# MAGPIE-ICL/synthPy

Hardware: AMD Instinct MI355X
Metric: ray-steps/sec (+ rays/sec to detector), 1e7 rays x 512^3 volume (higher is better)
Workload: dtype f64

## Files before the change

### include/synthray.h

```cpp
#ifndef SYNTHRAY_H
#define SYNTHRAY_H

#include <stddef.h>
#include <stdint.h>

#ifdef __cplusplus
extern "C" {
#endif

#define SR_OK 0
#define SR_ERR_INVALID (-1)
#define SR_ERR_HIP (-2)
#define SR_ERR_RCCL (-3)
#define SR_ERR_STATE (-4)

typedef struct sr_volume sr_volume;
typedef struct sr_rays sr_rays;
typedef struct sr_image sr_image;
typedef struct sr_comm sr_comm;

int sr_init(int device);
int sr_device_count(void);
int sr_synchronize(void);
int sr_device_memory(int64_t *free_bytes, int64_t *total_bytes);
// ... 176 lines not shown

int sr_ray_to_jones(const double *sf, int64_t n_rays, double extent, int probing_axis, int row_order,
                    double *rf, double *Jf);

int sr_rays_create(sr_rays **out, int64_t n_rays);
int sr_rays_upload(sr_rays *r, const double *s0);
int sr_rays_upload_part(sr_rays *r, const double *s0, int64_t n, int64_t first, int last);
int sr_rays_generate(sr_rays *r, int beam_type, double size_a, double size_b, double divergence, double ne_extent,
                     int probing_axis, uint64_t seed, uint64_t first_ray);
int sr_rays_trace(sr_rays *r, const sr_volume *v, const sr_trace_params *p, sr_trace_stats *stats);
int sr_rays_trace_stats(sr_rays *r, sr_trace_stats *stats);

int sr_rays_tile_segments(const sr_rays *r);
int sr_rays_tile_records(const sr_rays *r);
int sr_rays_launch_order(const sr_rays *r, uint32_t *order);
int sr_rays_set_count(sr_rays *r, int64_t n);
double sr_tile_min_density(void);
int sr_rays_download(const sr_rays *r, double *sf, double *rf, double *Jf);
int sr_rays_download_s0(const sr_rays *r, double *s0);
int sr_rays_error_bound(const sr_rays *r, float *bound);
int64_t sr_rays_count(const sr_rays *r);
int sr_rays_handoff_download(const sr_rays *r, double *rec);
int sr_rays_set_bbox(sr_rays *r, const double *bbox);
int sr_rays_get_bbox(const sr_rays *r, double *bbox, int *known);
int sr_rays_handoff_upload(sr_rays *r, const double *rec);
int sr_rays_handoff_send(sr_rays *r, sr_comm *comm, int peer);
int sr_rays_handoff_recv(sr_rays *r, sr_comm *comm, int peer);
void sr_rays_destroy(sr_rays *r);

enum {
// ... 86 lines not shown
```

### synthpy_amd/_ffi.py

```python
from __future__ import annotations

import ctypes as C
import os

import numpy as np

_HERE = os.path.dirname(os.path.abspath(__file__))
LIB_PATH = os.environ.get("SYNTHRAY_LIB") or os.path.join(_HERE, "libsynthray.so")


class SynthrayError(RuntimeError):
    """A libsynthray call returned a negative status."""


class Optic(C.Structure):
    _fields_ = [("op", C.c_int32), ("iarg", C.c_int32), ("a", C.c_double), ("b", C.c_double)]


class TraceParams(C.Structure):
    _fields_ = [("t_end", C.c_double), ("extent", C.c_double), ("dt", C.c_double), ("probing_axis", C.c_int32),
                ("row_order", C.c_int32), ("substeps", C.c_int32), ("sort_rays", C.c_int32), ("precision", C.c_int32),
                ("handoff", C.c_int32)]


# ... 127 lines not shown
    "sr_trace": (_i, [_vp, _vp, _i64, C.POINTER(TraceParams), _vp, _vp, _vp, C.POINTER(TraceStats)]),
    "sr_ray_to_jones": (_i, [_vp, _i64, _d, _i, _i, _vp, _vp]),
    "sr_rays_create": (_i, [_pp, _i64]),
    "sr_rays_download_s0": (_i, [_vp, _vp]),
    "sr_rays_error_bound": (_i, [_vp, _vp]),
    "sr_rays_generate": (_i, [_vp, _i, _d, _d, _d, _d, _i, C.c_uint64, C.c_uint64]),
    "sr_rays_upload": (_i, [_vp, _vp]),
    "sr_rays_upload_part": (_i, [_vp, _vp, _i64, _i64, _i]),
    "sr_rays_trace": (_i, [_vp, _vp, C.POINTER(TraceParams), C.POINTER(TraceStats)]),
    "sr_release_caches": (_i, []),
    "sr_rays_trace_stats": (_i, [_vp, C.POINTER(TraceStats)]),
    "sr_rays_tile_segments": (_i, [_vp]),
    "sr_tile_min_density": (_d, []),
    "sr_rays_tile_records": (_i, [_vp]),
    "sr_rays_launch_order": (_i, [_vp, _vp]),
    "sr_rays_set_count": (_i, [_vp, _i64]),
    "sr_rays_set_bbox": (_i, [_vp, _vp]),
    "sr_rays_get_bbox": (_i, [_vp, _vp, C.POINTER(C.c_int)]),
    "sr_rays_download": (_i, [_vp, _vp, _vp, _vp]),
    "sr_rays_count": (_i64, [_vp]),
    "sr_rays_destroy": (None, [_vp]),
    "sr_optics": (_i, [C.POINTER(Optic), _i, _d, _i64, _vp, _vp, _vp, _vp]),
    "sr_hist2d": (_i, [_vp, _vp, _i64, _i, _i, _d, _d, _d, _d, _vp]),
    "sr_interferogram": (_i, [_vp, _vp, _vp, _i64, _i, _i, _d, _d, _d, _d, _vp, _vp]),
    "sr_interfere_ref_beam": (_i, [_vp, _vp, _i64, _d, _d, _vp]),
    "sr_image_create": (_i, [_pp, _i, _i, _i, _d, _d, _d, _d]),
    "sr_image_zero": (_i, [_vp]),
    "sr_image_download": (_i, [_vp, _vp]),
    "sr_image_amplitude": (_i, [_vp, _vp]),
    "sr_image_counts_f64": (_i, [_vp, _vp]),
# ... 58 lines not shown
```

### synthpy_amd/csrc/common.hpp

```cpp
#pragma once
#include <hip/hip_runtime.h>

#include <algorithm>
#include <cmath>
#include <cstdarg>
#include <cstdint>
#include <cstdio>
#include <initializer_list>
#include <map>
#include <string>
#include <type_traits>
#include <vector>

#include "synthray.h"

namespace sr {

constexpr double kC = 299792458.0;

void set_error(const char *fmt, ...);
int fail(int code, const char *fmt, ...);

#define SR_HIP(call)                                                                         \
  do {                                                                                       \
// ... 178 lines not shown
  bool bbox_given = false;
  double *s0 = nullptr;
  double *sf = nullptr;
  double *rf = nullptr;
  double *Jf = nullptr;
  uint32_t *perm = nullptr;
  uint32_t *keys = nullptr;
  uint32_t *bins = nullptr;
  uint32_t *sort_tmp = nullptr;
  int64_t bins_cap = 0;
  uint32_t *fb_list = nullptr;
  unsigned long long *counters = nullptr;
  double *rec = nullptr;
  double *rec2 = nullptr;
  uint32_t *order2 = nullptr;
  double *strag_rec = nullptr;
  unsigned long long *strag_snap = nullptr;
  int strag_snap_cap = 0;
  bool have_s0 = false, traced = false, sorted = false, have_rec = false;
  bool have_order = false;
  bool counters_carry = false;
  int tile_segs = 0;
  int tile_segs_run = 0;
  bool tile_rec = false;
  float *guard = nullptr;
  const sr_volume *last_vol = nullptr;
  sr_trace_params last_p{};
  void *guard_set = nullptr;
  std::vector<char> guard_set_host;
  bool guard_live = false;
// ... 68 lines not shown
```

### synthpy_amd/csrc/trace.hip

```cpp
#include <algorithm>
#include <cmath>
#include <cstdlib>
#include <cstring>

#include "common.hpp"

namespace {

struct VolDev {
  const float4 *P;
  const float *L;
  const double *g[3];
  const double *rg[3];
  int na, nb, nc;
  double omega;
  const double *K;
  const double *Q;
  double verdet;
  int64_t OS;
  const double *R;
};

constexpr int64_t kSC = 8;
__device__ __forceinline__ int64_t col8(const VolDev &V, int ib, int ic) { return ((int64_t)ib * V.nc + ic) * 8; }
__device__ __forceinline__ int64_t koff(const VolDev &V, int k) { return (int64_t)(k >> 3) * V.OS + (k & 7); }

__device__ __forceinline__ void lds_dma16(const char *src, unsigned lane_off, unsigned dst) {
#ifdef SR_TILE_EXP_DMA_SADDR
  unsigned keep;
  asm volatile("s_mov_b32 %0, m0\n\ts_mov_b32 m0, %3\n\ts_nop 0\n\tglobal_load_lds_dwordx4 %1, %2\n\ts_mov_b32 m0, %0"
               : "=&s"(keep)
               : "v"(lane_off), "s"(src), "s"(dst)
               : "memory");
#else
  __builtin_amdgcn_global_load_lds((const __attribute__((address_space(1))) void *)(src + lane_off),
// ... 620 lines not shown
  V.P = v->P;
  V.L = v->L;
  for (int k = 0; k < 3; ++k) {
    V.g[k] = v->g[k];
    V.rg[k] = v->rg[k];
  }
  V.na = v->na;
  V.nb = v->nb;
  V.nc = v->nc;
  V.omega = v->omega;
  V.K = v->K;
  V.Q = v->Q;
  V.verdet = v->verdet;
  V.OS = (int64_t)v->nb * v->nc * 8;
  V.R = v->R;
  return V;
}

int bin_rays(sr_rays *r, int64_t N, int lo_bits, int n_coarse, uint32_t *out, hipStream_t st) {
  SR_CHECK(lo_bits <= 11 && n_coarse <= kBinMaxDigits + 1, "lateral grid too large for the LDS counters of the ray binning");
  const unsigned n_wg = (unsigned)((N + kBinTile - 1) / kBinTile);
  const int64_t ncount = (int64_t)n_coarse * n_wg;
  const int64_t nsb = (ncount + kScanPerBlock - 1) / kScanPerBlock;
  if (r->bins_cap < ncount + nsb) {
    sr::dev_free(r->bins);
    r->bins = nullptr;
    r->bins_cap = 0;
    int rc = sr::dev_alloc(&r->bins, (size_t)(ncount + nsb));
    if (rc) return rc;
    r->bins_cap = ncount + nsb;
// ... 4 lines not shown
  }
  uint32_t *sums = r->bins + ncount, *tkeys = r->sort_tmp, *trays = r->sort_tmp + N;
  hipLaunchKernelGGL(k_bin_count, dim3(n_wg), dim3(256), 0, st, (const uint32_t *)r->keys, N, lo_bits, n_coarse, r->bins, n_wg);
  hipLaunchKernelGGL(k_scan_blocks, dim3((unsigned)nsb), dim3(256), 0, st, r->bins, ncount, sums);
  hipLaunchKernelGGL(k_scan, dim3(1), dim3(1024), 0, st, sums, nsb);
  hipLaunchKernelGGL(k_scan_add, dim3(sr::grid_for(ncount, 256)), dim3(256), 0, st, r->bins, ncount, (const uint32_t *)sums);
  hipLaunchKernelGGL(k_bin_coarse, dim3(n_wg), dim3(256), 0, st, (const uint32_t *)r->keys, N, lo_bits, n_coarse,
                     (const uint32_t *)r->bins, n_wg, tkeys, trays);
  hipLaunchKernelGGL(k_bin_fine, dim3((unsigned)n_coarse), dim3(1024), 0, st, (const uint32_t *)tkeys, (const uint32_t *)trays, N,
                     lo_bits, n_coarse, (const uint32_t *)r->bins, n_wg, out);
  return SR_OK;
}

int bin_by_band(sr_rays *r, const sr_volume *v, const TileGeom &g, const double *rec, uint32_t *out, hipStream_t st) {
  const int64_t N = r->n;
  const int64_t n_bands = (v->nb - 1 + g.band - 1) / g.band;
  const int64_t n_keys = n_bands * (int64_t)(v->nc - 1) * g.band;
  int bits = 1;
  while (((int64_t)1 << bits) < n_keys) ++bits;
  const int shift = std::max(0, bits - 22);
  const int64_t key_max = ((n_keys - 1) >> shift) + 1;
  bits = 1;
  while (((int64_t)1 << bits) <= key_max) ++bits;
  const int lo_bits = std::min(11, (bits + 1) / 2);
  const int n_coarse = (int)(key_max >> lo_bits) + 1;
  SR_CHECK(n_coarse <= kBinMaxDigits + 1, "band key of %lld does not fit the LDS counters of the ray binning", (long long)key_max);
  const unsigned nblk = sr::grid_for(N, 256);
  if (rec)
    hipLaunchKernelGGL(k_keys_band_rec, dim3(nblk), dim3(256), 0, st, vol_dev(v), rec, N, g.band, (uint32_t)key_max, shift, r->keys);
  else
    hipLaunchKernelGGL(k_keys_band, dim3(nblk), dim3(256), 0, st, vol_dev(v), (const double *)r->s0, N, v->axis, g.band, (uint32_t)key_max,
                       shift, r->keys);
  return bin_rays(r, N, lo_bits, n_coarse, out, st);
}

constexpr double kTileMinDensity = 8.0;
struct TilePlan {
  TileGeom g;
  int seg;
  bool rec;
};

struct TraceKnobs {
  int f64_tile = -1;
  bool tile_records = true;
  bool strag_beside = true;
  bool aux_one_pass = false;
// ... 90 lines not shown
  const int threads = SR_TILE_THREADS;
  if (p->substeps != 1 || !p->sort_rays) return false;
  const bool aux = v->K || v->Q;
  if (records && !aux && threads == 256 && v->nb - 1 >= 8 && v->nc - 1 >= 7) {
    tp.rec = true;
    tp.g.tc = 7;
    tp.g.band = std::min(6, std::max(4, tp.g.band + 1));
    tp.seg = tp.g.band >= 5 ? 103 : 128;
  }
  if (knobs.tile_seg > 0) {
    tp.g = knobs.tile;
    tp.seg = knobs.tile_seg;
    tp.rec = tp.rec && tp.g.tb == 8 && tp.g.tc <= 8;
  }
  if (v->nb - 1 < tp.g.tb || v->nc - 1 < tp.g.tc || v->na < 3) return false;
  if (aux && (tp.g.tb * tp.g.tc > 64 || threads < 128)) return false;
  {
    const int steps = v->na - 1, n_seg = (steps + tp.seg - 1) / tp.seg;
    if (tile_lds_bytes(tp.g, (steps + n_seg - 1) / n_seg + 1, aux, tp.rec) > (size_t)160 * 1024) return false;
  }
  return true;
}

void launch_planes64(const sr_volume *v, const sr_trace_params *p, const TraceKnobs &knobs, const TraceArgs &A, hipStream_t st);

std::vector<double> tile_cut_weights(int n_seg) {
  std::vector<double> w((size_t)n_seg, 1.0);
  for (int q = 0; q < n_seg; ++q) w[(size_t)q] = n_seg > 1 ? 1.3 - 0.6 * q / (n_seg - 1) : 1.0;
  return w;
}
// ... 109 lines not shown
    T.k0 = cut[(size_t)q];
    T.k1 = cut[(size_t)q + 1];
    T.first = q == 0 && !ho_enter;
    T.last = q + 1 == n_seg;
    if (T.first) {
      T.rec_in = nullptr;
      T.order = nullptr;
      T.A.rec = r->rec;
    } else {
      rc = bin_by_band(r, v, tp.g, r->rec, r->order2, st);
      if (rc) return rc;
      T.rec_in = r->rec;
      T.order = r->order2;
      T.A.rec = r->rec2;
    }
    if (timed) SR_HIP(hipEventRecord(c.ev[4 + 2 * q], st));
    if ((rc = launch_tile(T, phase, aux, tp.rec, lds, st))) return rc;
    if (timed) SR_HIP(hipEventRecord(c.ev[5 + 2 * q], st));
    hipLaunchKernelGGL(k_strag_snap, dim3(1), dim3(1), 0, st, (const unsigned long long *)strag_count, r->strag_snap, q, r->counters + 3);
    hipStream_t ss = st;
    if (knobs.strag_beside) {
      SR_HIP(hipEventRecord(ev_go, st));
      SR_HIP(hipStreamWaitEvent(side, ev_go, 0));
      ss = side;
    }
    launch_planes64(v, p, knobs, straggler_args(A, r, cap, q, T.k0, ho_exit), ss);
    if (!T.first) std::swap(r->rec, r->rec2);
  }
  if (knobs.strag_beside) {
    SR_HIP(hipEventRecord(ev_done, side));
// ... 232 lines not shown
  A.in_count = count;
  A.out_list = r->keys;
  A.out_count = r->counters + 5;
  launch_planes64(v, &p, knobs, A, st);
  launch_time(v, A, st);
  SR_HIP(hipGetLastError());
  return SR_OK;
}

extern "C" {

void sr_rays_destroy(sr_rays *r) {
  if (!r) return;
  for (void *q : {(void *)r->s0, (void *)r->sf, (void *)r->rf, (void *)r->Jf, (void *)r->perm, (void *)r->keys, (void *)r->bins,
                  (void *)r->sort_tmp, (void *)r->fb_list, (void *)r->counters, (void *)r->rec, (void *)r->rec2, (void *)r->order2,
                  (void *)r->strag_rec, (void *)r->strag_snap, (void *)r->guard, r->guard_set})
    sr::dev_free(q);
  delete r;
}

int sr_rays_create(sr_rays **out, int64_t n) {
  SR_CHECK(out != nullptr, "sr_rays_create: NULL out");
  *out = nullptr;
  SR_CHECK(n >= 0 && n < (int64_t)0xFFFFFFFFll, "sr_rays_create: ray count %lld out of range", (long long)n);
  int rc = sr::ensure_init();
  if (rc) return rc;
  sr_rays *r = new sr_rays();
  r->n = n;
  r->cap = n;
  const size_t m = (size_t)(n > 0 ? n : 1);
  if ((rc = sr::dev_alloc(&r->s0, 9 * m)) || (rc = sr::dev_alloc(&r->sf, 9 * m)) || (rc = sr::dev_alloc(&r->rf, 4 * m)) ||
// ... 182 lines not shown

int sr_rays_tile_segments(const sr_rays *r) { return r ? r->tile_segs_run : 0; }

int sr_rays_tile_records(const sr_rays *r) { return r && r->tile_rec ? 1 : 0; }

int sr_rays_launch_order(const sr_rays *r, uint32_t *order) {
  SR_CHECK(r && order, "sr_rays_launch_order: NULL argument");
  if (!r->have_order) return sr::fail(SR_ERR_STATE, "sr_rays_launch_order: no trace has been queued for these rays");
  if (r->n == 0) return SR_OK;
  hipStream_t st = sr::ctx().stream;
  SR_HIP(hipMemcpyAsync(order, r->perm, sizeof(uint32_t) * (size_t)r->n, hipMemcpyDeviceToHost, st));
  SR_HIP(hipStreamSynchronize(st));
  return SR_OK;
}

int sr_rays_set_count(sr_rays *r, int64_t n) {
  SR_CHECK(r != nullptr, "sr_rays_set_count: NULL rays");
  SR_CHECK(n >= 0 && n <= r->cap, "sr_rays_set_count: %lld rays in a bundle made for %lld", (long long)n, (long long)r->cap);
  r->n = n;
  r->have_s0 = r->traced = r->sorted = r->have_rec = r->have_order = false;
  r->have_bbox = r->bbox_given = false;
  r->guard_live = false;
  r->last_vol = nullptr;
  r->tile_segs = r->tile_segs_run = 0;
  r->tile_rec = false;
  return SR_OK;
}

double sr_tile_min_density(void) { return kTileMinDensity; }

int sr_rays_download(const sr_rays *r, double *sf, double *rf, double *Jf) {
  SR_CHECK(r != nullptr, "sr_rays_download: NULL rays");
  return sr::download_rows(r, sf, rf, Jf, r->n, 0, nullptr);
}

// ... 113 lines not shown
```

### synthpy_amd/csrc/trace_tile.inc

```
struct TileGeom {
  int tb, tc;
  int halo;
  int band;
};

struct TileArgs {
  TraceArgs A;
  TileGeom G;
  int k0, k1;
  int first, last;
  int exit_rec, slab;
  int rot;
  unsigned block0;
  const double *rec_in;
  const uint32_t *order;
  uint32_t *perm_out;
  double *strag_rec;
  int64_t strag_cap;
  unsigned long long *strag_count;
};

constexpr int kRecColD = (1024 + 80) / 8;
__host__ __device__ constexpr int tile_rec(bool aux, bool rec = false) { return aux ? 38 : (rec ? 16 : 18); }

constexpr int kTabLo = 4, kTabHi = 5;
__host__ __device__ constexpr int tile_tab_entries(int t) { return kTabLo + t + kTabHi; }
__host__ __device__ constexpr int tile_tab_doubles(int tb, int tc) { return 2 * tile_tab_entries(tb) + 2 * tile_tab_entries(tc) + 4; }
static_assert(tile_tab_doubles(8, 8) * sizeof(double) <= 1024, "the records kernel's table head is one KiB");

__host__ __device__ inline size_t tile_lds_bytes(const TileGeom &g, int seg_steps, bool aux = false, bool rec = false) {
  const size_t tables = (size_t)(rec ? tile_tab_doubles(8, 8) : tile_tab_doubles(g.tb, g.tc));
  (void)seg_steps;
  const size_t head = rec ? (((tables * sizeof(double)) + 1023) & ~(size_t)1023) / sizeof(double) : ((tables + 1) & ~(size_t)1);
  if (rec) return sizeof(double) * (head + (size_t)5 * g.tc * kRecColD);
  return sizeof(double) * (head + (size_t)5 * g.tb * g.tc * tile_rec(aux, rec));
}

__device__ __forceinline__ uint32_t band_key(int ib, int ic, int ncc, int band) {
  const int bnd = ib / band, row = ib - bnd * band;
  const int col = (bnd & 1) ? ncc - 1 - ic : ic;
  return ((uint32_t)bnd * (uint32_t)ncc + (uint32_t)col) * (uint32_t)band + (uint32_t)row;
}

__global__ void k_keys_band(VolDev V, const double *__restrict__ s0, int64_t N, int axis, int band, uint32_t oob_key, int shift,
                            uint32_t *__restrict__ keys) {
  const int64_t i = blockIdx.x * (int64_t)blockDim.x + threadIdx.x;
  if (i >= N) return;
  const int b = (axis + 1) % 3, c = (axis + 2) % 3;
  double pa = s0[axis * N + i], pb = s0[b * N + i], pc = s0[c * N + i];
  const double va = s0[(3 + axis) * N + i], vb = s0[(3 + b) * N + i], vc = s0[(3 + c) * N + i];
  const double ga0 = V.g[0][0];
  if (va > 0 && pa < ga0) {
    const double tau = (ga0 - pa) / va;
    pb = pb + vb * tau;
    pc = pc + vc * tau;
  }
  const double gb0 = V.g[1][0], gbL = V.g[1][V.nb - 1], gc0 = V.g[2][0], gcL = V.g[2][V.nc - 1];
  uint32_t key = oob_key;
  if (pb >= gb0 && pb <= gbL && pc >= gc0 && pc <= gcL) {
    const int ib = find_cell(V.g[1], V.nb, pb, gb0, (V.nb - 1) / (gbL - gb0));
    const int ic = find_cell(V.g[2], V.nc, pc, gc0, (V.nc - 1) / (gcL - gc0));
    key = band_key(ib, ic, V.nc - 1, band) >> shift;
  }
  keys[i] = key;
}

__global__ void k_keys_band_rec(VolDev V, const double *__restrict__ rec, int64_t N, int band, uint32_t oob_key, int shift,
                                uint32_t *__restrict__ keys) {
  const int64_t j = blockIdx.x * (int64_t)blockDim.x + threadIdx.x;
  if (j >= N) return;
  const double pb = rec[j], pc = rec[N + j], va = rec[2 * N + j];
  const double gb0 = V.g[1][0], gbL = V.g[1][V.nb - 1], gc0 = V.g[2][0], gcL = V.g[2][V.nc - 1];
  uint32_t key = oob_key;
  if (va > 0 && pb >= gb0 && pb <= gbL && pc >= gc0 && pc <= gcL) {
    const int ib = find_cell(V.g[1], V.nb, pb, gb0, (V.nb - 1) / (gbL - gb0));
    const int ic = find_cell(V.g[2], V.nc, pc, gc0, (V.nc - 1) / (gcL - gc0));
    key = band_key(ib, ic, V.nc - 1, band) >> shift;
  }
  keys[j] = key;
}

__global__ void k_strag_snap(const unsigned long long *count, unsigned long long *snap, int q, unsigned long long *total) {
  const unsigned long long c = *count;
  snap[q + 1] = c;
  *total += c - snap[q];
}

struct StragFinish {
  TraceArgs A;
  const double *strag;
  int64_t cap;
  int exit_rec, slab;
};
__global__ __launch_bounds__(256) void k_strag_finish(StragFinish F) {
// ... 58 lines not shown
  }
}

#ifndef SR_TILE_THREADS
#define SR_TILE_THREADS 256
#endif
#ifndef SR_TILE_WAVES
#define SR_TILE_WAVES 3
#endif
#ifndef SR_TILE_REC_WAVES
#define SR_TILE_REC_WAVES 4
#endif
template <bool PHASE, bool AUX = false, bool REC = false>
__global__ __launch_bounds__(SR_TILE_THREADS, AUX ? 2 : (REC ? SR_TILE_REC_WAVES : SR_TILE_WAVES)) void k_trace_tile(TileArgs T) {
  static_assert(!(AUX && REC), "the ready-made records hold the gradient fields only");
  constexpr int kTileRec = tile_rec(AUX, REC);
  extern __shared__ double lds[];
  const TraceArgs &A = T.A;
  const VolDev &V = A.V;
  const int TB = T.G.tb, TC = T.G.tc, NC = TB * TC;
  const int tab_nb = tile_tab_entries(REC ? 8 : TB), tab_nc = tile_tab_entries(REC ? 8 : TC);
  int *org = reinterpret_cast<int *>(lds + 2 * (tab_nb + tab_nc));
  const size_t tables = REC ? 1024 / sizeof(double) : ((size_t)tile_tab_doubles(TB, TC) + 1) & ~(size_t)1;
  const unsigned tab_b = (unsigned)(uintptr_t)(__attribute__((address_space(3))) double *)lds + kTabLo * 16u;
  const unsigned tab_c = tab_b + (unsigned)tab_nb * 16u;
  double *recs = lds + tables;
  const int slot_d = REC ? TC * kRecColD : NC * kTileRec;
  auto cell_off = [&](int b_, int c_) { return REC ? __mul24(c_, kRecColD * 8) + b_ * 16 : (c_ * TB + b_) * kTileRec; };

  const unsigned chunk = gridDim.x / 8;
// ... 18 lines not shown
    q6 = 0;
    const double ga0 = Q.V.g[0][0];
    bool ok = (q2 > 0) && (pa <= ga0);
    if (ok && pa < ga0) {
      const double tau = (ga0 - pa) / q2;
      if (tau >= Q.t_end) {
        ok = false;
      } else {
        q0 = q0 + q3 * tau;
        q1 = q1 + q4 * tau;
        q6 = tau;
      }
    }
    return ok;
  };
  if (T.first) {
    i = have ? (int64_t)A.perm[j] : 0;
    if (have) alive = from_s0(A, i, y0, y1, y2, y3, y4, y5, y6);
    if (AUX && have) {
      y7 = A.s0[6 * N + i];
      y8 = A.s0[8 * N + i];
    }
    if (!alive) y2 = 1;
  } else if (have) {
    const int64_t o = (int64_t)T.order[j];
    const double *R = T.rec_in;
    if (AUX) {
      y7 = R[7 * N + o];
      y8 = R[8 * N + o];
    } else {
      A.rec[7 * N + j] = R[7 * N + o];
      A.rec[8 * N + j] = R[8 * N + o];
    }
    y0 = R[o];
    y1 = R[N + o];
    y2 = R[2 * N + o];
    y3 = R[3 * N + o];
    y4 = R[4 * N + o];
    y5 = R[5 * N + o];
    y6 = R[6 * N + o];
    const double idx = R[9 * N + o];
    A.rec[9 * N + j] = idx;
    T.perm_out[j] = (uint32_t)idx;
    alive = y2 == y2;
  }
  const bool gone = have && !T.first && y2 == -__builtin_inf();
  alive = alive && (y0 == y0) && (y1 == y1) && (y3 == y3) && (y4 == y4) && (y5 == y5) && (y2 < 1e30) && (y2 > 1e-30);
  const bool entered = alive;

  int cb = 0, cc = 0, xb = 0, xc = 0;
  if (alive) {
    const double gb0 = V.g[1][0], gbL = V.g[1][V.nb - 1], gc0 = V.g[2][0], gcL = V.g[2][V.nc - 1];
    if (y0 >= gb0 && y0 < gbL && y1 >= gc0 && y1 < gcL) {
      const double rb0 = (V.nb - 1) / (gbL - gb0), rc0 = (V.nc - 1) / (gcL - gc0);
      cb = find_cell(V.g[1], V.nb, y0, gb0, rb0);
      cc = find_cell(V.g[2], V.nc, y1, gc0, rc0);
      const double dz = (V.g[0][T.k1] - V.g[0][T.k0]) / y2;
      const double eb = fmin(fmax(fma(y3, dz, y0), gb0), gbL), ec = fmin(fmax(fma(y4, dz, y1), gc0), gcL);
      xb = find_cell(V.g[1], V.nb, eb, gb0, rb0);
      xc = find_cell(V.g[2], V.nc, ec, gc0, rc0);
    } else {
      alive = false;
    }
  }
  if (threadIdx.x < 8) org[threadIdx.x] = (threadIdx.x & 2) ? -1 : 0x7fffffff;
  __syncthreads();
  if (alive) {
    atomicMin(&org[0], cb);
    atomicMin(&org[1], cc);
    atomicMax(&org[2], cb);
    atomicMax(&org[3], cc);
    atomicMin(&org[4], min(cb, xb));
    atomicMin(&org[5], min(cc, xc));
    atomicMax(&org[6], max(cb, xb));
    atomicMax(&org[7], max(cc, xc));
  }
  __syncthreads();
  auto place = [](int lo_e, int hi_e, int lo_x, int hi_x, int t, int cells) {
    if (hi_e < 0) return 0;
    int lo = lo_x, hi = hi_x;
    if (hi - lo + 1 > t) {
      lo = lo_e;
      hi = hi_e;
    }
    if (hi - lo + 1 > t) hi = lo + t - 1;
    return min(max(lo - (t - (hi - lo + 1)) / 2, 0), cells - t);
  };
  const int ob = place(org[0], org[2], org[4], org[6], TB, V.nb - 1), oc = place(org[1], org[3], org[5], org[7], TC, V.nc - 1);
  typedef double d2 __attribute__((ext_vector_type(2)));
  typedef __attribute__((address_space(3))) d2 *lds_d2_t;
  auto fill_table = [&](unsigned tab, int t_cells, const double *g, const double *rg, int o) {
    for (int t = threadIdx.x; t < tile_tab_entries(t_cells); t += blockDim.x) {
      const int n = t - kTabLo;
      d2 e = {n < 0 ? __builtin_inf() : -__builtin_inf(), 1.0};
      if (n >= 0 && n <= t_cells) e.x = g[o + n];
      if (n >= 0 && n < t_cells) e.y = rg[o + n];
      ((lds_d2_t)(uintptr_t)tab)[n] = e;
    }
  };
  fill_table(tab_b, TB, V.g[1], V.rg[1], ob);
  fill_table(tab_c, TC, V.g[2], V.rg[2], oc);
  __syncthreads();
  int tb = cb - ob, tc = cc - oc;
  if (alive && !(tb >= 0 && tb < TB && tc >= 0 && tc < TC)) alive = false;
  if (!alive) tb = tc = 0;
  double lo_b, r_b, lo_c, r_c;
  {
    const d2 eb = ((lds_d2_t)(uintptr_t)tab_b)[tb], ec = ((lds_d2_t)(uintptr_t)tab_c)[tc];
    lo_b = eb.x;
    r_b = eb.y;
    lo_c = ec.x;
    r_c = ec.y;
  }
  int cell = cell_off(tb, tc);

  const int p_first = T.rot ? (int)((blockIdx.x >> 8) & 3u) * 64 : 0;
  const int p_lane = (int)((threadIdx.x + blockDim.x - (unsigned)p_first % blockDim.x) % blockDim.x);
  const bool producer = !REC && wg_live && p_lane < NC;
  const int pcell = producer ? p_lane * kTileRec : 0;
  const int64_t sc = kSC, sb = (int64_t)V.nc * 8;
  const int64_t pcol = producer ? col8(V, ob + p_lane % TB, oc + p_lane / TB) : 0;
  struct RawPlane {
    float4 v[4];
    float l[4];
  };
  auto issue_raw = [&](int k, RawPlane &r) {
    const int64_t ko = koff(V, k);
    const float4 *q = V.P + pcol + ko;
// ... 77 lines not shown
    CoefPlane p, q;
    coefs_from_corners<PHASE>(r.v, r.l, p);
    store_rec(dst, pcell, p);
    if (prev >= 0) {
      load_rec(prev, pcell, q);
#pragma unroll
      for (int f = 0; f < 4; ++f) {
        q.a[f] += p.a[f];
        q.b[f] += p.b[f];
        q.c[f] += p.c[f];
        q.d[f] += p.d[f];
      }
      store_rec(mid, pcell, q);
    }
  };
  const int wv = __builtin_amdgcn_readfirstlane((int)(threadIdx.x >> 6));
  const int ln = (int)(threadIdx.x & 63);
  const int ob_u = __builtin_amdgcn_readfirstlane(ob), oc_u = __builtin_amdgcn_readfirstlane(oc);
  unsigned lane_off = (unsigned)(ln & 7) * 128u + (unsigned)(ln >> 3) * 16u;
  const int64_t col_bytes = (int64_t)(V.nb - 1) * 128, plane_bytes = (int64_t)(V.nc - 1) * col_bytes;
  const char *tile_r = REC ? reinterpret_cast<const char *>(V.R) + ((int64_t)oc_u * (V.nb - 1) + ob_u) * 128 : nullptr;
  const unsigned recs_lds = (unsigned)(uintptr_t)recs;
  auto slot_h = [&](int slot) { return REC ? (int)(recs_lds + (unsigned)(slot * slot_d) * 8u) : slot; };
  const int wcol_b = 2 * wv * (kRecColD * 8);
  const char *wcol_r = REC ? tile_r + (int64_t)(2 * wv) * col_bytes : nullptr;
  auto glds16 = [&](const char *src, int dst) { lds_dma16(src, lane_off, (unsigned)dst); };
  auto dma_cols = [&](const char *src0, const char *src1, int slot) {
    if (2 * wv < TC) glds16(src0, slot + wcol_b);
    if (2 * wv + 1 < TC) glds16(src1, slot + wcol_b + kRecColD * 8);
  };
  const int mid_lane = wcol_b + ln * 16;
  auto mid_from = [&](int lo, int hi, int mid, bool col0, bool col1) {
#pragma unroll
    for (int q = 0; q < 2; ++q) {
      if (!(q ? col1 : col0)) break;
      const d2 a = ((lds_d2_t)(uintptr_t)(unsigned)(lo + mid_lane))[q * (kRecColD / 2)];
      const d2 b = ((lds_d2_t)(uintptr_t)(unsigned)(hi + mid_lane))[q * (kRecColD / 2)];
      ((lds_d2_t)(uintptr_t)(unsigned)(mid + mid_lane))[q * (kRecColD / 2)] = a + b;
    }
  };
  if (REC && wg_live) {
    const char *p0 = wcol_r + (int64_t)T.k0 * plane_bytes;
    dma_cols(p0, p0 + col_bytes, slot_h(T.k0 % 3));
    dma_cols(p0 + plane_bytes, p0 + plane_bytes + col_bytes, slot_h((T.k0 + 1) % 3));
    asm volatile("s_waitcnt vmcnt(0)" ::: "memory");
    mid_from(slot_h(T.k0 % 3), slot_h((T.k0 + 1) % 3), slot_h(3 + T.k0 % 2), 2 * wv < TC, 2 * wv + 1 < TC);
  }
  if (producer) {
    RawPlane r0, r1;
    issue_raw(T.k0, r0);
    issue_raw(T.k0 + 1, r1);
    produce(r0, T.k0 % 3, -1, 0);
    produce(r1, (T.k0 + 1) % 3, T.k0 % 3, 3 + T.k0 % 2);
  }
  if (aproducer) {
    double u0[4][5], u1[4][5];
    aux_corners(V, apcol + koff(V, T.k0), u0);
    aux_corners(V, apcol + koff(V, T.k0 + 1), u1);
    produce_aux(u0, T.k0 % 3, -1, 0);
// ... 43 lines not shown
  asm volatile("s_waitcnt lgkmcnt(" #n ")"                                                                                      \
               : "+v"(R.q[0]), "+v"(R.q[1]), "+v"(R.q[2]), "+v"(R.q[3]), "+v"(R.q[4]), "+v"(R.q[5]), "+v"(R.q[6]), "+v"(R.q[7]))

  int s_lo = slot_h(T.k0 % 3), s_hi = slot_h((T.k0 + 1) % 3), s_nx = slot_h((T.k0 + 2) % 3);
  int m_cur = slot_h(3 + T.k0 % 2), m_nx = slot_h(3 + (T.k0 + 1) % 2);
  constexpr int kNever = -0x7fffffff - 1;
  const int k_col0 = (wg_live && 2 * wv < TC) ? T.k1 - 2 : kNever, k_col1 = (wg_live && 2 * wv + 1 < TC) ? T.k1 - 2 : kNever;
  const char *nx_r0 = REC ? wcol_r + (int64_t)(T.k0 + 2) * plane_bytes : nullptr, *nx_r1 = REC ? nx_r0 + col_bytes : nullptr;
  Rec RA, RB;
  request(s_lo, cell, RA);
  typedef const double __attribute__((address_space(4))) *cdbl_t;
  const cdbl_t ctab = (cdbl_t)(uintptr_t)A.tab64;
  const cdbl_t tab0 = ctab + 8 * (int64_t)T.k0;
  cdbl_t tab = tab0;
  double nh = tab[0], nhh = tab[1], nh6 = tab[2], nh6w = tab[6];
  for (int k = T.k0; k < T.k1; ++k) {
    const double Sh = nh, Shh = nhh, Sh6 = nh6, Sh6w = nh6w;
    {
      tab = k + 1 < T.k1 ? tab + 8 : tab0;
      nh = tab[0];
      nhh = tab[1];
      nh6 = tab[2];
      nh6w = tab[6];
    }
    RawPlane NX;
    double NXU[20];
    const bool more = k + 2 <= T.k1;
    const bool more0 = k <= k_col0, more1 = k <= k_col1;
#ifndef SR_TILE_EXP_NOPRODUCE
    if (REC) {
      if (more0) {
// ... 302 lines not shown
```

### synthpy_amd/engine.py

```python
from __future__ import annotations

import contextlib
import ctypes as C
import os
import weakref
from dataclasses import dataclass

import numpy as np

from . import _ffi
from ._ffi import check, f32, f64, lib, ptr

c = 299792458.0

OP_DIST, OP_LENS, OP_CIRC_AP, OP_CIRC_STOP, OP_RECT_AP, OP_KNIFE, OP_SCALE, OP_PHASE = range(8)
ROWS_LEGACY, ROWS_JAX = 0, 1
IMG_COUNTS, IMG_COMPLEX, IMG_INTENSITY = 0, 1, 2
VOL_PHASE = 1

_AXES = {"x": 0, "y": 1, "z": 2}


def axis_index(probing_direction) -> int:
    if isinstance(probing_direction, str) and probing_direction in _AXES:
# ... 732 lines not shown
        return TraceStats(st.ray_steps, st.fallback_rays, st.trace_kernel_ms, st.total_ms)

    @property
    def tile_segments(self) -> int:
        return int(lib.sr_rays_tile_segments(self._h))

    @property
    def tile_records(self) -> bool:
        return bool(lib.sr_rays_tile_records(self._h))

    def launch_order(self):
        out = np.empty(self.n, np.uint32)
        check(lib.sr_rays_launch_order(self._h, ptr(out)))
        return out

    def resize(self, n_rays: int):
        check(lib.sr_rays_set_count(self._h, int(n_rays)))
        self.n = int(n_rays)
        self.generation += 1
        return self

    @property
    def bbox(self):
        box, known = np.zeros(6), C.c_int(0)
        check(lib.sr_rays_get_bbox(self._h, ptr(box), C.byref(known)))
        return box if known.value else None

    @bbox.setter
    def bbox(self, box):
        check(lib.sr_rays_set_bbox(self._h, None if box is None else ptr(f64(np.asarray(box, dtype=np.float64).reshape(6)))))
# ... 277 lines not shown
```

Baseline: 126.0 billion.

## Reuse binned cell indices and replace LDS atomics with packed wave reductions in tile prologue

The band-binning key kernels now also store each ray's packed lateral cell (16 bits per axis), and the tile kernel reads it instead of searching the grid again with find_cell. The workgroup bounding box is computed with DPP wave reductions on packed u16 min/max and a small per-wave LDS scratch, replacing eight LDS atomics and one barrier. The lateral table fill moves after the DMA issue so it overlaps the record loads. The cost is an extra device buffer and global read per ray, a 65535-cell lateral limit, and a cell that is stale if positions drift from the binned ones (clamped but possibly wrong).

New measurement: 132.5 billion (median of 6 runs). 1.05x the previous value.

```diff
diff --git a/include/synthray.h b/include/synthray.h
--- a/include/synthray.h
+++ b/include/synthray.h
@@ -214,6 +214,7 @@
 int sr_rays_tile_segments(const sr_rays *r);
 int sr_rays_tile_records(const sr_rays *r);
 int sr_rays_launch_order(const sr_rays *r, uint32_t *order);
+int sr_rays_binned_cells(const sr_rays *r, uint32_t *cells);
 int sr_rays_set_count(sr_rays *r, int64_t n);
 double sr_tile_min_density(void);
 int sr_rays_download(const sr_rays *r, double *sf, double *rf, double *Jf);
diff --git a/synthpy_amd/_ffi.py b/synthpy_amd/_ffi.py
--- a/synthpy_amd/_ffi.py
+++ b/synthpy_amd/_ffi.py
@@ -165,6 +165,7 @@
     "sr_tile_min_density": (_d, []),
     "sr_rays_tile_records": (_i, [_vp]),
     "sr_rays_launch_order": (_i, [_vp, _vp]),
+    "sr_rays_binned_cells": (_i, [_vp, _vp]),
     "sr_rays_set_count": (_i, [_vp, _i64]),
     "sr_rays_set_bbox": (_i, [_vp, _vp]),
     "sr_rays_get_bbox": (_i, [_vp, _vp, C.POINTER(C.c_int)]),
diff --git a/synthpy_amd/csrc/common.hpp b/synthpy_amd/csrc/common.hpp
--- a/synthpy_amd/csrc/common.hpp
+++ b/synthpy_amd/csrc/common.hpp
@@ -216,6 +216,8 @@
   double *rec = nullptr;
   double *rec2 = nullptr;
   uint32_t *order2 = nullptr;
+  uint32_t *cells = nullptr;
+  bool have_cells = false;
   double *strag_rec = nullptr;
   unsigned long long *strag_snap = nullptr;
   int strag_snap_cap = 0;
diff --git a/synthpy_amd/csrc/trace.hip b/synthpy_amd/csrc/trace.hip
--- a/synthpy_amd/csrc/trace.hip
+++ b/synthpy_amd/csrc/trace.hip
@@ -19,6 +19,7 @@
   double verdet;
   int64_t OS;
   const double *R;
+  double rb0, rc0;
 };
 
 constexpr int64_t kSC = 8;
@@ -669,6 +670,8 @@
   V.verdet = v->verdet;
   V.OS = (int64_t)v->nb * v->nc * 8;
   V.R = v->R;
+  V.rb0 = v->hg[1].size() > 1 ? (v->nb - 1) / (v->hg[1].back() - v->hg[1].front()) : 0.0;
+  V.rc0 = v->hg[2].size() > 1 ? (v->nc - 1) / (v->hg[2].back() - v->hg[2].front()) : 0.0;
   return V;
 }
 
@@ -703,6 +706,12 @@
 
 int bin_by_band(sr_rays *r, const sr_volume *v, const TileGeom &g, const double *rec, uint32_t *out, hipStream_t st) {
   const int64_t N = r->n;
+  SR_CHECK(v->nb - 1 <= 0xFFFF && v->nc - 1 <= 0xFFFF, "lateral grid of %d x %d cells: a packed cell holds 16 bits per axis", v->nb - 1, v->nc - 1);
+  if (!r->cells) {
+    int rc = sr::dev_alloc(&r->cells, (size_t)std::max<int64_t>(std::max(r->cap, N), 1));
+    if (rc) return rc;
+  }
+  r->have_cells = true;
   const int64_t n_bands = (v->nb - 1 + g.band - 1) / g.band;
   const int64_t n_keys = n_bands * (int64_t)(v->nc - 1) * g.band;
   int bits = 1;
@@ -716,10 +725,10 @@
   SR_CHECK(n_coarse <= kBinMaxDigits + 1, "band key of %lld does not fit the LDS counters of the ray binning", (long long)key_max);
   const unsigned nblk = sr::grid_for(N, 256);
   if (rec)
-    hipLaunchKernelGGL(k_keys_band_rec, dim3(nblk), dim3(256), 0, st, vol_dev(v), rec, N, g.band, (uint32_t)key_max, shift, r->keys);
+    hipLaunchKernelGGL(k_keys_band_rec, dim3(nblk), dim3(256), 0, st, vol_dev(v), rec, N, g.band, (uint32_t)key_max, shift, r->keys, r->cells);
   else
     hipLaunchKernelGGL(k_keys_band, dim3(nblk), dim3(256), 0, st, vol_dev(v), (const double *)r->s0, N, v->axis, g.band, (uint32_t)key_max,
-                       shift, r->keys);
+                       shift, r->keys, r->cells);
   return bin_rays(r, N, lo_bits, n_coarse, out, st);
 }
 
@@ -840,6 +849,7 @@
     tp.rec = tp.rec && tp.g.tb == 8 && tp.g.tc <= 8;
   }
   if (v->nb - 1 < tp.g.tb || v->nc - 1 < tp.g.tc || v->na < 3) return false;
+  if (v->nb - 1 > 0xFFFF || v->nc - 1 > 0xFFFF) return false;
   if (aux && (tp.g.tb * tp.g.tc > 64 || threads < 128)) return false;
   {
     const int steps = v->na - 1, n_seg = (steps + tp.seg - 1) / tp.seg;
@@ -979,6 +989,8 @@
       T.order = r->order2;
       T.A.rec = r->rec2;
     }
+    SR_CHECK(r->cells != nullptr, "tile path: the rays were not binned by band before the launch");
+    T.cells = r->cells;
     if (timed) SR_HIP(hipEventRecord(c.ev[4 + 2 * q], st));
     if ((rc = launch_tile(T, phase, aux, tp.rec, lds, st))) return rc;
     if (timed) SR_HIP(hipEventRecord(c.ev[5 + 2 * q], st));
@@ -1241,7 +1253,7 @@
   if (!r) return;
   for (void *q : {(void *)r->s0, (void *)r->sf, (void *)r->rf, (void *)r->Jf, (void *)r->perm, (void *)r->keys, (void *)r->bins,
                   (void *)r->sort_tmp, (void *)r->fb_list, (void *)r->counters, (void *)r->rec, (void *)r->rec2, (void *)r->order2,
-                  (void *)r->strag_rec, (void *)r->strag_snap, (void *)r->guard, r->guard_set})
+                  (void *)r->strag_rec, (void *)r->strag_snap, (void *)r->guard, r->guard_set, (void *)r->cells})
     sr::dev_free(q);
   delete r;
 }
@@ -1454,11 +1466,21 @@
   return SR_OK;
 }
 
+int sr_rays_binned_cells(const sr_rays *r, uint32_t *cells) {
+  SR_CHECK(r && cells, "sr_rays_binned_cells: NULL argument");
+  if (!r->have_cells) return sr::fail(SR_ERR_STATE, "sr_rays_binned_cells: the tile path has not binned these rays");
+  if (r->n == 0) return SR_OK;
+  hipStream_t st = sr::ctx().stream;
+  SR_HIP(hipMemcpyAsync(cells, r->cells, sizeof(uint32_t) * (size_t)r->n, hipMemcpyDeviceToHost, st));
+  SR_HIP(hipStreamSynchronize(st));
+  return SR_OK;
+}
+
 int sr_rays_set_count(sr_rays *r, int64_t n) {
   SR_CHECK(r != nullptr, "sr_rays_set_count: NULL rays");
   SR_CHECK(n >= 0 && n <= r->cap, "sr_rays_set_count: %lld rays in a bundle made for %lld", (long long)n, (long long)r->cap);
   r->n = n;
-  r->have_s0 = r->traced = r->sorted = r->have_rec = r->have_order = false;
+  r->have_s0 = r->traced = r->sorted = r->have_rec = r->have_order = r->have_cells = false;
   r->have_bbox = r->bbox_given = false;
   r->guard_live = false;
   r->last_vol = nullptr;
diff --git a/synthpy_amd/csrc/trace_tile.inc b/synthpy_amd/csrc/trace_tile.inc
--- a/synthpy_amd/csrc/trace_tile.inc
+++ b/synthpy_amd/csrc/trace_tile.inc
@@ -15,6 +15,7 @@
   const double *rec_in;
   const uint32_t *order;
   uint32_t *perm_out;
+  const uint32_t *cells;
   double *strag_rec;
   int64_t strag_cap;
   unsigned long long *strag_count;
@@ -25,7 +26,7 @@
 
 constexpr int kTabLo = 4, kTabHi = 5;
 __host__ __device__ constexpr int tile_tab_entries(int t) { return kTabLo + t + kTabHi; }
-__host__ __device__ constexpr int tile_tab_doubles(int tb, int tc) { return 2 * tile_tab_entries(tb) + 2 * tile_tab_entries(tc) + 4; }
+__host__ __device__ constexpr int tile_tab_doubles(int tb, int tc) { return 2 * tile_tab_entries(tb) + 2 * tile_tab_entries(tc) + 32; }
 static_assert(tile_tab_doubles(8, 8) * sizeof(double) <= 1024, "the records kernel's table head is one KiB");
 
 __host__ __device__ inline size_t tile_lds_bytes(const TileGeom &g, int seg_steps, bool aux = false, bool rec = false) {
@@ -36,14 +37,38 @@
   return sizeof(double) * (head + (size_t)5 * g.tb * g.tc * tile_rec(aux, rec));
 }
 
+typedef unsigned short pk_u16 __attribute__((ext_vector_type(2)));
+__device__ __forceinline__ unsigned pk_min_u16(unsigned a, unsigned b) {
+  return __builtin_bit_cast(unsigned, __builtin_elementwise_min(__builtin_bit_cast(pk_u16, a), __builtin_bit_cast(pk_u16, b)));
+}
+__device__ __forceinline__ unsigned pk_max_u16(unsigned a, unsigned b) {
+  return __builtin_bit_cast(unsigned, __builtin_elementwise_max(__builtin_bit_cast(pk_u16, a), __builtin_bit_cast(pk_u16, b)));
+}
+template <int CTRL, int ROWS>
+__device__ __forceinline__ unsigned dpp_from(unsigned v) {
+  return (unsigned)__builtin_amdgcn_update_dpp((int)v, (int)v, CTRL, ROWS, 0xf, false);
+}
+template <bool MAX>
+__device__ __forceinline__ unsigned wave_pk_u16(unsigned v) {
+  auto op = [](unsigned a, unsigned b) { return MAX ? pk_max_u16(a, b) : pk_min_u16(a, b); };
+  v = op(v, dpp_from<0xB1, 0xf>(v));
+  v = op(v, dpp_from<0x4E, 0xf>(v));
+  v = op(v, dpp_from<0x141, 0xf>(v));
+  v = op(v, dpp_from<0x140, 0xf>(v));
+  v = op(v, dpp_from<0x142, 0xa>(v));
+  v = op(v, dpp_from<0x143, 0xc>(v));
+  return v;
+}
+
 __device__ __forceinline__ uint32_t band_key(int ib, int ic, int ncc, int band) {
   const int bnd = ib / band, row = ib - bnd * band;
   const int col = (bnd & 1) ? ncc - 1 - ic : ic;
   return ((uint32_t)bnd * (uint32_t)ncc + (uint32_t)col) * (uint32_t)band + (uint32_t)row;
 }
 
+constexpr uint32_t kNoCell = 0xFFFFFFFFu;
 __global__ void k_keys_band(VolDev V, const double *__restrict__ s0, int64_t N, int axis, int band, uint32_t oob_key, int shift,
-                            uint32_t *__restrict__ keys) {
+                            uint32_t *__restrict__ keys, uint32_t *__restrict__ cells) {
   const int64_t i = blockIdx.x * (int64_t)blockDim.x + threadIdx.x;
   if (i >= N) return;
   const int b = (axis + 1) % 3, c = (axis + 2) % 3;
@@ -56,28 +81,32 @@
     pc = pc + vc * tau;
   }
   const double gb0 = V.g[1][0], gbL = V.g[1][V.nb - 1], gc0 = V.g[2][0], gcL = V.g[2][V.nc - 1];
-  uint32_t key = oob_key;
+  uint32_t key = oob_key, cell = kNoCell;
   if (pb >= gb0 && pb <= gbL && pc >= gc0 && pc <= gcL) {
-    const int ib = find_cell(V.g[1], V.nb, pb, gb0, (V.nb - 1) / (gbL - gb0));
-    const int ic = find_cell(V.g[2], V.nc, pc, gc0, (V.nc - 1) / (gcL - gc0));
+    const int ib = find_cell(V.g[1], V.nb, pb, gb0, V.rb0);
+    const int ic = find_cell(V.g[2], V.nc, pc, gc0, V.rc0);
     key = band_key(ib, ic, V.nc - 1, band) >> shift;
+    cell = (uint32_t)ib | ((uint32_t)ic << 16);
   }
   keys[i] = key;
+  cells[i] = cell;
 }
 
 __global__ void k_keys_band_rec(VolDev V, const double *__restrict__ rec, int64_t N, int band, uint32_t oob_key, int shift,
-                                uint32_t *__restrict__ keys) {
+                                uint32_t *__restrict__ keys, uint32_t *__restrict__ cells) {
   const int64_t j = blockIdx.x * (int64_t)blockDim.x + threadIdx.x;
   if (j >= N) return;
   const double pb = rec[j], pc = rec[N + j], va = rec[2 * N + j];
   const double gb0 = V.g[1][0], gbL = V.g[1][V.nb - 1], gc0 = V.g[2][0], gcL = V.g[2][V.nc - 1];
-  uint32_t key = oob_key;
+  uint32_t key = oob_key, cell = kNoCell;
   if (va > 0 && pb >= gb0 && pb <= gbL && pc >= gc0 && pc <= gcL) {
-    const int ib = find_cell(V.g[1], V.nb, pb, gb0, (V.nb - 1) / (gbL - gb0));
-    const int ic = find_cell(V.g[2], V.nc, pc, gc0, (V.nc - 1) / (gcL - gc0));
+    const int ib = find_cell(V.g[1], V.nb, pb, gb0, V.rb0);
+    const int ic = find_cell(V.g[2], V.nc, pc, gc0, V.rc0);
     key = band_key(ib, ic, V.nc - 1, band) >> shift;
+    cell = (uint32_t)ib | ((uint32_t)ic << 16);
   }
   keys[j] = key;
+  cells[j] = cell;
 }
 
 __global__ void k_strag_snap(const unsigned long long *count, unsigned long long *snap, int q, unsigned long long *total) {
@@ -166,6 +195,7 @@
 template <bool PHASE, bool AUX = false, bool REC = false>
 __global__ __launch_bounds__(SR_TILE_THREADS, AUX ? 2 : (REC ? SR_TILE_REC_WAVES : SR_TILE_WAVES)) void k_trace_tile(TileArgs T) {
   static_assert(!(AUX && REC), "the ready-made records hold the gradient fields only");
+  static_assert(SR_TILE_THREADS % 64 == 0 && SR_TILE_THREADS / 64 <= 16, "the placement's scratch holds one slot per wavefront, 16 at the most");
   constexpr int kTileRec = tile_rec(AUX, REC);
   extern __shared__ double lds[];
   const TraceArgs &A = T.A;
@@ -214,8 +244,10 @@
     }
     return ok;
   };
+  uint32_t pk = kNoCell;
   if (T.first) {
     i = have ? (int64_t)A.perm[j] : 0;
+    if (have) pk = T.cells[i];
     if (have) alive = from_s0(A, i, y0, y1, y2, y3, y4, y5, y6);
     if (AUX && have) {
       y7 = A.s0[6 * N + i];
@@ -225,6 +257,7 @@
   } else if (have) {
     const int64_t o = (int64_t)T.order[j];
     const double *R = T.rec_in;
+    pk = T.cells[o];
     if (AUX) {
       y7 = R[7 * N + o];
       y8 = R[8 * N + o];
@@ -248,36 +281,50 @@
   alive = alive && (y0 == y0) && (y1 == y1) && (y3 == y3) && (y4 == y4) && (y5 == y5) && (y2 < 1e30) && (y2 > 1e-30);
   const bool entered = alive;
 
+  const int wv = __builtin_amdgcn_readfirstlane((int)(threadIdx.x >> 6));
+  const int ln = (int)(threadIdx.x & 63);
   int cb = 0, cc = 0, xb = 0, xc = 0;
+  double lo_b = 0, r_b = 1, lo_c = 0, r_c = 1;
   if (alive) {
     const double gb0 = V.g[1][0], gbL = V.g[1][V.nb - 1], gc0 = V.g[2][0], gcL = V.g[2][V.nc - 1];
-    if (y0 >= gb0 && y0 < gbL && y1 >= gc0 && y1 < gcL) {
-      const double rb0 = (V.nb - 1) / (gbL - gb0), rc0 = (V.nc - 1) / (gcL - gc0);
-      cb = find_cell(V.g[1], V.nb, y0, gb0, rb0);
-      cc = find_cell(V.g[2], V.nc, y1, gc0, rc0);
-      const double dz = (V.g[0][T.k1] - V.g[0][T.k0]) / y2;
-      const double eb = fmin(fmax(fma(y3, dz, y0), gb0), gbL), ec = fmin(fmax(fma(y4, dz, y1), gc0), gcL);
-      xb = find_cell(V.g[1], V.nb, eb, gb0, rb0);
-      xc = find_cell(V.g[2], V.nc, ec, gc0, rc0);
+    if (y0 >= gb0 && y0 < gbL && y1 >= gc0 && y1 < gcL && pk != kNoCell) {
+      cb = min((int)(pk & 0xffffu), V.nb - 2);
+      cc = min((int)(pk >> 16), V.nc - 2);
+      lo_b = V.g[1][cb];
+      r_b = V.rg[1][cb];
+      lo_c = V.g[2][cc];
+      r_c = V.rg[2][cc];
+      const double dz = (V.g[0][T.k1] - V.g[0][T.k0]) * rcp_f64_from_f32(y2);
+      const double ub = fma(y3 * dz, r_b, (y0 - lo_b) * r_b), uc = fma(y4 * dz, r_c, (y1 - lo_c) * r_c);
+      xb = min(max(cb + (int)floor(fmin(fmax(ub, -65536.0), 65536.0)), 0), V.nb - 2);
+      xc = min(max(cc + (int)floor(fmin(fmax(uc, -65536.0), 65536.0)), 0), V.nc - 2);
     } else {
       alive = false;
     }
   }
-  if (threadIdx.x < 8) org[threadIdx.x] = (threadIdx.x & 2) ? -1 : 0x7fffffff;
+  uint4 *box = reinterpret_cast<uint4 *>(org);
+  {
+    unsigned e = 0xFFFFFFFFu, x = 0xFFFFFFFFu, E = 0u, X = 0u;
+    if (alive) {
+      e = E = (unsigned)cb | ((unsigned)cc << 16);
+      x = (unsigned)min(cb, xb) | ((unsigned)min(cc, xc) << 16);
+      X = (unsigned)max(cb, xb) | ((unsigned)max(cc, xc) << 16);
+    }
+    e = wave_pk_u16<false>(e);
+    x = wave_pk_u16<false>(x);
+    E = wave_pk_u16<true>(E);
+    X = wave_pk_u16<true>(X);
+    if (ln == 63) box[wv] = make_uint4(e, x, E, X);
+  }
   __syncthreads();
-  if (alive) {
-    atomicMin(&org[0], cb);
-    atomicMin(&org[1], cc);
-    atomicMax(&org[2], cb);
-    atomicMax(&org[3], cc);
-    atomicMin(&org[4], min(cb, xb));
-    atomicMin(&org[5], min(cc, xc));
-    atomicMax(&org[6], max(cb, xb));
-    atomicMax(&org[7], max(cc, xc));
-  }
-  __syncthreads();
+  uint4 bx = box[0];
+#pragma unroll
+  for (int w = 1; w < SR_TILE_THREADS / 64; ++w) {
+    const uint4 o = box[w];
+    bx = make_uint4(pk_min_u16(bx.x, o.x), pk_min_u16(bx.y, o.y), pk_max_u16(bx.z, o.z), pk_max_u16(bx.w, o.w));
+  }
   auto place = [](int lo_e, int hi_e, int lo_x, int hi_x, int t, int cells) {
-    if (hi_e < 0) return 0;
+    if (hi_e < lo_e) return 0;
     int lo = lo_x, hi = hi_x;
     if (hi - lo + 1 > t) {
       lo = lo_e;
@@ -286,7 +333,8 @@
     if (hi - lo + 1 > t) hi = lo + t - 1;
     return min(max(lo - (t - (hi - lo + 1)) / 2, 0), cells - t);
   };
-  const int ob = place(org[0], org[2], org[4], org[6], TB, V.nb - 1), oc = place(org[1], org[3], org[5], org[7], TC, V.nc - 1);
+  const int ob = place((int)(bx.x & 0xffffu), (int)(bx.z & 0xffffu), (int)(bx.y & 0xffffu), (int)(bx.w & 0xffffu), TB, V.nb - 1);
+  const int oc = place((int)(bx.x >> 16), (int)(bx.z >> 16), (int)(bx.y >> 16), (int)(bx.w >> 16), TC, V.nc - 1);
   typedef double d2 __attribute__((ext_vector_type(2)));
   typedef __attribute__((address_space(3))) d2 *lds_d2_t;
   auto fill_table = [&](unsigned tab, int t_cells, const double *g, const double *rg, int o) {
@@ -298,20 +346,9 @@
       ((lds_d2_t)(uintptr_t)tab)[n] = e;
     }
   };
-  fill_table(tab_b, TB, V.g[1], V.rg[1], ob);
-  fill_table(tab_c, TC, V.g[2], V.rg[2], oc);
-  __syncthreads();
   int tb = cb - ob, tc = cc - oc;
   if (alive && !(tb >= 0 && tb < TB && tc >= 0 && tc < TC)) alive = false;
   if (!alive) tb = tc = 0;
-  double lo_b, r_b, lo_c, r_c;
-  {
-    const d2 eb = ((lds_d2_t)(uintptr_t)tab_b)[tb], ec = ((lds_d2_t)(uintptr_t)tab_c)[tc];
-    lo_b = eb.x;
-    r_b = eb.y;
-    lo_c = ec.x;
-    r_c = ec.y;
-  }
   int cell = cell_off(tb, tc);
 
   const int p_first = T.rot ? (int)((blockIdx.x >> 8) & 3u) * 64 : 0;
@@ -419,8 +456,6 @@
       store_rec(mid, pcell, q);
     }
   };
-  const int wv = __builtin_amdgcn_readfirstlane((int)(threadIdx.x >> 6));
-  const int ln = (int)(threadIdx.x & 63);
   const int ob_u = __builtin_amdgcn_readfirstlane(ob), oc_u = __builtin_amdgcn_readfirstlane(oc);
   unsigned lane_off = (unsigned)(ln & 7) * 128u + (unsigned)(ln >> 3) * 16u;
   const int64_t col_bytes = (int64_t)(V.nb - 1) * 128, plane_bytes = (int64_t)(V.nc - 1) * col_bytes;
@@ -448,6 +483,10 @@
     const char *p0 = wcol_r + (int64_t)T.k0 * plane_bytes;
     dma_cols(p0, p0 + col_bytes, slot_h(T.k0 % 3));
     dma_cols(p0 + plane_bytes, p0 + plane_bytes + col_bytes, slot_h((T.k0 + 1) % 3));
+  }
+  fill_table(tab_b, TB, V.g[1], V.rg[1], ob);
+  fill_table(tab_c, TC, V.g[2], V.rg[2], oc);
+  if (REC && wg_live) {
     asm volatile("s_waitcnt vmcnt(0)" ::: "memory");
     mid_from(slot_h(T.k0 % 3), slot_h((T.k0 + 1) % 3), slot_h(3 + T.k0 % 2), 2 * wv < TC, 2 * wv + 1 < TC);
   }
@@ -521,7 +560,12 @@
   const cdbl_t tab0 = ctab + 8 * (int64_t)T.k0;
   cdbl_t tab = tab0;
   double nh = tab[0], nhh = tab[1], nh6 = tab[2], nh6w = tab[6];
-  for (int k = T.k0; k < T.k1; ++k) {
+#ifdef SR_TILE_EXP_NOSTEPS
+  const int k_stop = T.k0;
+#else
+  const int k_stop = T.k1;
+#endif
+  for (int k = T.k0; k < k_stop; ++k) {
     const double Sh = nh, Shh = nhh, Sh6 = nh6, Sh6w = nh6w;
     {
       tab = k + 1 < T.k1 ? tab + 8 : tab0;
diff --git a/synthpy_amd/engine.py b/synthpy_amd/engine.py
--- a/synthpy_amd/engine.py
+++ b/synthpy_amd/engine.py
@@ -770,6 +770,13 @@
         check(lib.sr_rays_launch_order(self._h, ptr(out)))
         return out
 
+    def binned_cells(self):
+        out = np.empty(self.n, np.uint32)
+        check(lib.sr_rays_binned_cells(self._h, ptr(out)))
+        cells = np.stack([out & 0xFFFF, out >> 16]).astype(np.int64)
+        cells[:, out == 0xFFFFFFFF] = -1
+        return cells
+
     def resize(self, n_rays: int):
         check(lib.sr_rays_set_count(self._h, int(n_rays)))
         self.n = int(n_rays)
```
